# MiniMax-AI/VTP

Measured on AMD Instinct MI355X. Metric: images/sec/node VTP-B f16d64 256x256 train step, higher is better.
Workload: dtype bf16

## Files before the change

### vtp_amd/csrc/attention_resident.hip

```cpp
#include "common.h"
#include "diag.h"
#include <algorithm>
#include <cstdio>
#include "vtp_hip.h"

namespace vtp {

constexpr float LOG2E_R = 1.4426950408889634f;
constexpr float LN2_R = 0.6931471805599453f;
constexpr int RES_MAXN = 320;
constexpr int RES_SPLIT_COLS = 4;

struct AttnResArgs {
  const bf16 *q, *k, *v, *o, *d_o;
  bf16 *out, *dq, *dk, *dv;
  float* lse;
  float* delta;
  const bf16 *rope_sin, *rope_cos;
  int rope_prefix;
  int B, N, heads, npad;
  long sb, sn, sbo, sno;
  float scale;
  int stagger;
  unsigned long long* timing;
};

__device__ __forceinline__ void attn_stamp(const AttnResArgs& p, size_t wg, int lane, int wave, int i) {
  if (__builtin_expect(p.timing != nullptr, 0) && lane == 0) diag_stamp(p.timing, (wg * 16 + wave) * 8 + i);
}
__device__ __forceinline__ int grid_wg() { return (blockIdx.z * gridDim.y + blockIdx.y) * gridDim.x + blockIdx.x; }

__device__ __forceinline__ int swz_key(int r) { return (((r >> 1) & 1) << 2) | ((r >> 2) & 3); }

__device__ __forceinline__ void stage_resident(const bf16* __restrict__ base, long sn, int N, int npad, char* lds, int wave,
                                               int nwaves, int lane) {
  const int rr = lane >> 3, cp = lane & 7;
  for (int piece = wave; piece < (npad >> 3); piece += nwaves) {
    const int row = piece * 8 + rr;
    const int c = cp ^ swz_key(row);
    const bf16* src = base + (long)min(row, N - 1) * sn + c * 8;
    __builtin_amdgcn_global_load_lds((const __attribute__((address_space(1))) void*)src,
                                     (__attribute__((address_space(3))) void*)(lds + piece * 1024), 16, 0, 0);
  }
}

__device__ __forceinline__ bf16x8 frag_row(const char* lds, int row0, int ks, int lane) {
  const int r = row0 + (lane & 31);
  return *(const bf16x8*)(lds + r * 128 + (((2 * ks + (lane >> 5)) ^ swz_key(r)) << 4));
}
__device__ __forceinline__ bf16x8 frag_tr(const char* lds, int dblk, int row0, int ks, int lane) {
  const int i = lane & 15, g = (lane >> 4) & 1, hi = lane >> 5;
  const int r = row0 + ks * 16 + hi * 4 + (i >> 2);
  const int col = dblk * 32 + g * 16 + (i & 3) * 4;
  const char* p0 = lds + r * 128 + (((col >> 3) ^ swz_key(r)) << 4) + ((col & 7) << 1);
  const char* p1 = lds + (r + 8) * 128 + (((col >> 3) ^ swz_key(r + 8)) << 4) + ((col & 7) << 1);
  bf16x4 lo = __builtin_amdgcn_ds_read_tr16_b64_v4bf16((__attribute__((address_space(3))) bf16x4*)p0);
  bf16x4 hi4 = __builtin_amdgcn_ds_read_tr16_b64_v4bf16((__attribute__((address_space(3))) bf16x4*)p1);
  return __builtin_shufflevector(lo, hi4, 0, 1, 2, 3, 4, 5, 6, 7);
}

__device__ __forceinline__ int row_part(int lane) {
  const int r = lane & 31;
  return r * 128 + (((lane >> 5) ^ swz_key(r)) << 4);
}
__device__ __forceinline__ int tr_part(int lane, int half) {
  const int i = lane & 15, g = (lane >> 4) & 1, hi = lane >> 5;
  const int r = hi * 4 + (i >> 2) + 8 * half;
  const int col = g * 16 + (i & 3) * 4;
  return r * 128 + (((col >> 3) ^ swz_key(r)) << 4) + ((col & 7) << 1);
}
__device__ __forceinline__ int lds_addr(int lane_part, int uniform_part) {
  int a;
  asm("v_add_u32 %0, %1, %2" : "=v"(a) : "s"(uniform_part), "v"(lane_part));
  return a;
}
__device__ __forceinline__ bf16x8 frag_row_at(int addr) { return *(const __attribute__((address_space(3))) bf16x8*)(size_t)addr; }
__device__ __forceinline__ bf16x8 frag_tr_at(int addr0, int addr1, int ks) {
  bf16x4 lo = __builtin_amdgcn_ds_read_tr16_b64_v4bf16((__attribute__((address_space(3))) bf16x4*)(size_t)(addr0 + ks * 2048));
  bf16x4 hi4 = __builtin_amdgcn_ds_read_tr16_b64_v4bf16((__attribute__((address_space(3))) bf16x4*)(size_t)(addr1 + ks * 2048));
  return __builtin_shufflevector(lo, hi4, 0, 1, 2, 3, 4, 5, 6, 7);
}

__device__ __forceinline__ bf16x8 pack8r(const f32x16& a, int base) {
  f32x4 x = {a[base], a[base + 1], a[base + 2], a[base + 3]}, y = {a[base + 4], a[base + 5], a[base + 6], a[base + 7]};
  bf16x4 xb = __builtin_convertvector(x, bf16x4), yb = __builtin_convertvector(y, bf16x4);
  return __builtin_shufflevector(xb, yb, 0, 1, 2, 3, 4, 5, 6, 7);
}
__device__ __forceinline__ void zero16r(f32x16& a) {
#pragma unroll
  for (int r = 0; r < 16; ++r) a[r] = 0.f;
}
__device__ __forceinline__ void wait_all_dma() { asm volatile("s_waitcnt vmcnt(0)" ::: "memory"); }
__device__ __forceinline__ void wait_vmcnt_upto(int n) {
  switch (n) {
    case 0: asm volatile("s_waitcnt vmcnt(0)" ::: "memory"); break;
    case 1: asm volatile("s_waitcnt vmcnt(1)" ::: "memory"); break;
    case 2: asm volatile("s_waitcnt vmcnt(2)" ::: "memory"); break;
    case 3: asm volatile("s_waitcnt vmcnt(3)" ::: "memory"); break;
    case 4: asm volatile("s_waitcnt vmcnt(4)" ::: "memory"); break;
    case 5: asm volatile("s_waitcnt vmcnt(5)" ::: "memory"); break;
    case 6: asm volatile("s_waitcnt vmcnt(6)" ::: "memory"); break;
    case 7: asm volatile("s_waitcnt vmcnt(7)" ::: "memory"); break;
    case 8: asm volatile("s_waitcnt vmcnt(8)" ::: "memory"); break;
    case 9: asm volatile("s_waitcnt vmcnt(9)" ::: "memory"); break;
    case 10: asm volatile("s_waitcnt vmcnt(10)" ::: "memory"); break;
    case 11: asm volatile("s_waitcnt vmcnt(11)" ::: "memory"); break;
    case 12: asm volatile("s_waitcnt vmcnt(12)" ::: "memory"); break;
    case 13: asm volatile("s_waitcnt vmcnt(13)" ::: "memory"); break;
    case 14: asm volatile("s_waitcnt vmcnt(14)" ::: "memory"); break;
    case 15: asm volatile("s_waitcnt vmcnt(15)" ::: "memory"); break;
    case 16: asm volatile("s_waitcnt vmcnt(16)" ::: "memory"); break;
    case 17: asm volatile("s_waitcnt vmcnt(17)" ::: "memory"); break;
    case 18: asm volatile("s_waitcnt vmcnt(18)" ::: "memory"); break;
    case 19: asm volatile("s_waitcnt vmcnt(19)" ::: "memory"); break;
    case 20: asm volatile("s_waitcnt vmcnt(20)" ::: "memory"); break;
    case 21: asm volatile("s_waitcnt vmcnt(21)" ::: "memory"); break;
    case 22: asm volatile("s_waitcnt vmcnt(22)" ::: "memory"); break;
    case 23: asm volatile("s_waitcnt vmcnt(23)" ::: "memory"); break;
    case 24: asm volatile("s_waitcnt vmcnt(24)" ::: "memory"); break;
    case 25: asm volatile("s_waitcnt vmcnt(25)" ::: "memory"); break;
    case 26: asm volatile("s_waitcnt vmcnt(26)" ::: "memory"); break;
    case 27: asm volatile("s_waitcnt vmcnt(27)" ::: "memory"); break;
    case 28: asm volatile("s_waitcnt vmcnt(28)" ::: "memory"); break;
    case 29: asm volatile("s_waitcnt vmcnt(29)" ::: "memory"); break;
    case 30: asm volatile("s_waitcnt vmcnt(30)" ::: "memory"); break;
    case 31: asm volatile("s_waitcnt vmcnt(31)" ::: "memory"); break;
    case 32: asm volatile("s_waitcnt vmcnt(32)" ::: "memory"); break;
    default: asm volatile("s_waitcnt vmcnt(0)" ::: "memory"); break;
  }
}

__device__ __forceinline__ void store_grad_pair(bf16* row, int d0, f32x4 lo, f32x4 hi, const bf16* sin_t, const bf16* cos_t, long t) {
  bf16x4 a4 = __builtin_convertvector(lo, bf16x4), b4 = __builtin_convertvector(hi, bf16x4);
  if (sin_t) {
    const bf16x4 c1 = *(const bf16x4*)(cos_t + t + d0), c2 = *(const bf16x4*)(cos_t + t + d0 + 32);
    const bf16x4 s1 = *(const bf16x4*)(sin_t + t + d0), s2 = *(const bf16x4*)(sin_t + t + d0 + 32);
    bf16x4 o1, o2;
#pragma unroll
    for (int e = 0; e < 4; ++e) {
      const float a = bf2f(a4[e]), b = bf2f(b4[e]);
      o1[e] = f2bf(bf2f(f2bf(a * bf2f(c1[e]))) + bf2f(f2bf(b * bf2f(s2[e]))));
      o2[e] = f2bf(bf2f(f2bf(b * bf2f(c2[e]))) + bf2f(f2bf(-a * bf2f(s1[e]))));
    }
    a4 = o1;
    b4 = o2;
  }
  *(bf16x4*)(row + d0) = a4;
  *(bf16x4*)(row + d0 + 32) = b4;
}

__global__ __launch_bounds__(640) void attn_fwd_res_kernel(const AttnResArgs p) {
  extern __shared__ __attribute__((aligned(16))) char smem[];
  char* Ks = smem;
  char* Vs = smem + p.npad * 128;
  const int lane = threadIdx.x & 63, wave = __builtin_amdgcn_readfirstlane(threadIdx.x >> 6), nwaves = blockDim.x >> 6, hi = lane >> 5;
  const int h = blockIdx.x, b = blockIdx.y;
// ... 534 lines not shown
      dk[db] = __builtin_amdgcn_mfma_f32_32x32x16_bf16(frag_tr_at(tq0, tq1, 0), d0, dk[db], 0, 0, 0);
      dk[db] = __builtin_amdgcn_mfma_f32_32x32x16_bf16(frag_tr_at(tq0, tq1, 1), d1, dk[db], 0, 0, 0);
    }
  }
  stamp(2);
  if (ki < p.N) {
  bf16* krow = p.dk + (long)b * p.sb + (long)ki * p.sn + h * 64;
  bf16* vrow = p.dv + (long)b * p.sb + (long)ki * p.sn + h * 64;
  const bool rot = p.rope_sin && ki >= p.rope_prefix;
  const long t = (long)(ki - p.rope_prefix) * 64;
#pragma unroll
  for (int g = 0; g < 4; ++g) {
    f32x4 lo, hv, c0, c1;
#pragma unroll
    for (int e = 0; e < 4; ++e) {
      lo[e] = dk[0][4 * g + e];
      hv[e] = dk[1][4 * g + e];
      c0[e] = dv[0][4 * g + e];
      c1[e] = dv[1][4 * g + e];
    }
    store_grad_pair(krow, 8 * g + 4 * hi, lo, hv, rot ? p.rope_sin : nullptr, p.rope_cos, t);
    store_grad_pair(vrow, 8 * g + 4 * hi, c0, c1, nullptr, nullptr, 0);
  }
  }
  stamp(3);
}

constexpr int PB_WAVES = 8;
constexpr int PB_XROWS = 2;

__device__ __forceinline__ int stage_image_asm(const bf16* base, long sn, int N, int npad, unsigned img_off, int wave, int nwaves,
                                               int lane) {
  int n = 0;
  for (int piece = wave; piece < (npad >> 3); piece += nwaves, ++n) stage_piece_asm(base, sn, N, piece, img_off, lane);
  return n;
}

__device__ __forceinline__ void dq_step(const bf16x8 (&qf)[4], const bf16x8 (&dof)[4], f32x16 (&dq)[2], const int (&rpart)[4],
                                        const int (&tpart)[2][2], int koff, int img, f32x2 sc2v, f32x2 nlse, f32x2 scv, f32x2 ndlt,
                                        int key0, int N, bool mask, int hi) {
  f32x16 s, dp;
  zero16r(s);
  zero16r(dp);
#pragma unroll
  for (int ks = 0; ks < 4; ++ks) {
    s = __builtin_amdgcn_mfma_f32_32x32x16_bf16(frag_row_at(lds_addr(rpart[ks], koff)), qf[ks], s, 0, 0, 0);
    dp = __builtin_amdgcn_mfma_f32_32x32x16_bf16(frag_row_at(lds_addr(rpart[ks], koff + img)), dof[ks], dp, 0, 0, 0);
  }
#pragma unroll
  for (int i = 0; i < 8; ++i) {
    f32x2 e = {s[2 * i], s[2 * i + 1]}, g = {dp[2 * i], dp[2 * i + 1]};
    e = __builtin_elementwise_fma(e, sc2v, nlse);
    g = __builtin_elementwise_fma(g, scv, ndlt);
    e[0] = fast_exp2(e[0]);
    e[1] = fast_exp2(e[1]);
    e *= g;
    s[2 * i] = e[0];
    s[2 * i + 1] = e[1];
  }
  if (mask) {
#pragma unroll
    for (int r = 0; r < 16; ++r)
      if (key0 + (r & 3) + 8 * (r >> 2) + 4 * hi >= N) s[r] = 0.f;
  }
  const bf16x8 d0 = pack8r(s, 0), d1 = pack8r(s, 8);
#pragma unroll
  for (int db = 0; db < 2; ++db) {
    const int t0 = lds_addr(tpart[db][0], koff), t1 = lds_addr(tpart[db][1], koff);
    dq[db] = __builtin_amdgcn_mfma_f32_32x32x16_bf16(frag_tr_at(t0, t1, 0), d0, dq[db], 0, 0, 0);
    dq[db] = __builtin_amdgcn_mfma_f32_32x32x16_bf16(frag_tr_at(t0, t1, 1), d1, dq[db], 0, 0, 0);
  }
}

__device__ __forceinline__ float row_delta(const bf16x8 (&of)[4], const bf16x8 (&dof)[4]) {
  float dlt = 0.f;
#pragma unroll
  for (int ks = 0; ks < 4; ++ks)
#pragma unroll
    for (int e = 0; e < 8; ++e) dlt += bf2f(of[ks][e]) * bf2f(dof[ks][e]);
  return dlt + __shfl_xor(dlt, 32, 64);
}

__device__ __forceinline__ void dkv_step(const bf16x8 (&kf)[4], const bf16x8 (&vf)[4], f32x16 (&dk)[2], f32x16 (&dv)[2],
                                         const int (&rpart)[4], const int (&tpart)[2][2], int qoff, int img, const float* lse_s,
                                         const float* dlt_s, f32x2 sc2v, f32x2 scv, int q0, int N, bool mask, int hi) {
  f32x16 s, dp;
  zero16r(s);
  zero16r(dp);
#pragma unroll
  for (int ks = 0; ks < 4; ++ks) {
    s = __builtin_amdgcn_mfma_f32_32x32x16_bf16(frag_row_at(lds_addr(rpart[ks], qoff)), kf[ks], s, 0, 0, 0);
    dp = __builtin_amdgcn_mfma_f32_32x32x16_bf16(frag_row_at(lds_addr(rpart[ks], qoff + img)), vf[ks], dp, 0, 0, 0);
  }
  f32x16 pr;
#pragma unroll
  for (int g = 0; g < 4; ++g) {
    const f32x4 l4 = *(const f32x4*)(lse_s + q0 + 8 * g + 4 * hi);
    const f32x4 d4 = *(const f32x4*)(dlt_s + q0 + 8 * g + 4 * hi);
#pragma unroll
    for (int e2 = 0; e2 < 2; ++e2) {
      const int r = 4 * g + 2 * e2;
      f32x2 e = {s[r], s[r + 1]}, gq = {dp[r], dp[r + 1]};
      e = __builtin_elementwise_fma(e, sc2v, f32x2{l4[2 * e2], l4[2 * e2 + 1]});
      gq = __builtin_elementwise_fma(gq, scv, f32x2{d4[2 * e2], d4[2 * e2 + 1]});
      e[0] = fast_exp2(e[0]);
      e[1] = fast_exp2(e[1]);
      if (mask) {
        if (q0 + 8 * g + 4 * hi + 2 * e2 >= N) e[0] = 0.f;
        if (q0 + 8 * g + 4 * hi + 2 * e2 + 1 >= N) e[1] = 0.f;
      }
      pr[r] = e[0];
      pr[r + 1] = e[1];
      e *= gq;
      s[r] = e[0];
      s[r + 1] = e[1];
    }
  }
  const bf16x8 p0 = pack8r(pr, 0), p1 = pack8r(pr, 8), d0 = pack8r(s, 0), d1 = pack8r(s, 8);
#pragma unroll
  for (int db = 0; db < 2; ++db) {
    const int tq0 = lds_addr(tpart[db][0], qoff), tq1 = lds_addr(tpart[db][1], qoff);
    const int tg0 = lds_addr(tpart[db][0], qoff + img), tg1 = lds_addr(tpart[db][1], qoff + img);
    dv[db] = __builtin_amdgcn_mfma_f32_32x32x16_bf16(frag_tr_at(tg0, tg1, 0), p0, dv[db], 0, 0, 0);
    dv[db] = __builtin_amdgcn_mfma_f32_32x32x16_bf16(frag_tr_at(tg0, tg1, 1), p1, dv[db], 0, 0, 0);
    dk[db] = __builtin_amdgcn_mfma_f32_32x32x16_bf16(frag_tr_at(tq0, tq1, 0), d0, dk[db], 0, 0, 0);
    dk[db] = __builtin_amdgcn_mfma_f32_32x32x16_bf16(frag_tr_at(tq0, tq1, 1), d1, dk[db], 0, 0, 0);
  }
}

__device__ __forceinline__ void put_slot(float* slot, const f32x16 (&acc)[2], int hi) {
#pragma unroll
  for (int db = 0; db < 2; ++db)
#pragma unroll
    for (int g = 0; g < 4; ++g) {
      f32x4 v;
#pragma unroll
      for (int e = 0; e < 4; ++e) v[e] = acc[db][4 * g + e];
      *(f32x4*)(slot + 32 * db + 8 * g + 4 * hi) = v;
    }
}
__device__ __forceinline__ void store_acc_rows(bf16* row, const f32x16 (&acc)[2], int hi, const bf16* sin_t, const bf16* cos_t, long t) {
#pragma unroll
  for (int g = 0; g < 4; ++g) {
    f32x4 lo, hv;
#pragma unroll
    for (int e = 0; e < 4; ++e) {
      lo[e] = acc[0][4 * g + e];
      hv[e] = acc[1][4 * g + e];
    }
    store_grad_pair(row, 8 * g + 4 * hi, lo, hv, sin_t, cos_t, t);
  }
}

template <int W>
__global__ __launch_bounds__(64 * W) void attn_bwd_fused_kernel(const AttnResArgs p) {
  extern __shared__ __attribute__((aligned(16))) char smem[];
  const int lane = threadIdx.x & 63, wave = threadIdx.x >> 6, hi = lane >> 5;
  const int img = p.npad * 128, nb = p.npad >> 5, last = nb - 1;
  const bool odd = nb > W;
  const int nx = odd ? p.N - 32 * W : 0;
  const int QO = 0, KO = img, VO = 2 * img, GO = 3 * img;
  float* lse_s = (float*)(smem + 4 * img);
  float* dlt_s = lse_s + p.npad;
  float* xq = dlt_s + p.npad;
  float* xk = xq + (W + 1) * PB_XROWS * 64;
  float* xv = xk + (W + 1) * PB_XROWS * 64;
  const int hid = blockIdx.x, b = hid / p.heads, h = hid - b * p.heads;
  auto stamp = [&p, lane, wave, hid](int i) { attn_stamp(p, hid, lane, wave, i); };
  stamp(0);
  stage_image_asm(p.q + (long)b * p.sb + h * 64, p.sn, p.N, p.npad, QO, wave, W, lane);
  stage_image_asm(p.d_o + (long)b * p.sbo + h * 64, p.sno, p.N, p.npad, GO, wave, W, lane);
  stage_image_asm(p.k + (long)b * p.sb + h * 64, p.sn, p.N, p.npad, KO, wave, W, lane);
  stage_image_asm(p.v + (long)b * p.sb + h * 64, p.sn, p.N, p.npad, VO, wave, W, lane);
  const float sc2 = p.scale * LOG2E_R;
  const f32x2 sc2v = {sc2, sc2}, scv = {p.scale, p.scale};
  int rpart[4], tpart[2][2];
#pragma unroll
  for (int ks = 0; ks < 4; ++ks) rpart[ks] = row_part(lane) ^ (ks << 5);
#pragma unroll
  for (int db = 0; db < 2; ++db)
#pragma unroll
    for (int hf = 0; hf < 2; ++hf) tpart[db][hf] = tr_part(lane, hf) ^ (db << 6);
  const long srow0 = ((long)b * p.heads + h) * p.N;
  const int ri = wave * 32 + (lane & 31);
  const int rx = 32 * W + (lane & 31);
  bf16x8 of[4], of2[4];
  float lse_raw, lse_raw2 = 0.f;
  {
    const int qc = min(ri, p.N - 1);
    const bf16* orow = p.o + (long)b * p.sbo + h * 64 + (long)qc * p.sno + hi * 8;
#pragma unroll
    for (int ks = 0; ks < 4; ++ks) of[ks] = *(const bf16x8*)(orow + ks * 16);
    lse_raw = p.lse[srow0 + qc];
    if (odd) {
      const int qc2 = min(rx, p.N - 1);
      const bf16* orow2 = p.o + (long)b * p.sbo + h * 64 + (long)qc2 * p.sno + hi * 8;
#pragma unroll
      for (int ks = 0; ks < 4; ++ks) of2[ks] = *(const bf16x8*)(orow2 + ks * 16);
      lse_raw2 = p.lse[srow0 + qc2];
    }
  }
  wait_all_dma();
  __syncthreads();
  stamp(1);
  {
    bf16x8 qf[4], dof[4];
    const int own = __builtin_amdgcn_readfirstlane(wave * 4096);
#pragma unroll
    for (int ks = 0; ks < 4; ++ks) {
      qf[ks] = frag_row_at(lds_addr(rpart[ks], QO + own));
      dof[ks] = frag_row_at(lds_addr(rpart[ks], GO + own));
    }
    const float dlt = row_delta(of, dof);
    if (hi == 0) {
      lse_s[ri] = -lse_raw * LOG2E_R;
      dlt_s[ri] = -dlt * p.scale;
      if (ri < p.N) p.delta[srow0 + ri] = dlt;
    }
    {
      const float lse2 = lse_raw * LOG2E_R;
      const f32x2 nlse = {-lse2, -lse2}, ndlt = {-dlt * p.scale, -dlt * p.scale};
      f32x16 dq[2];
      zero16r(dq[0]);
      zero16r(dq[1]);
      for (int kb = 0; kb < nb; ++kb)
        dq_step(qf, dof, dq, rpart, tpart, __builtin_amdgcn_readfirstlane(KO + kb * 4096), img, sc2v, nlse, scv, ndlt, kb * 32, p.N,
                kb == last && (p.N & 31), hi);
      if (ri < p.N) {
        const bool rot = p.rope_sin && ri >= p.rope_prefix;
        store_acc_rows(p.dq + (long)b * p.sb + (long)ri * p.sn + h * 64, dq, hi, rot ? p.rope_sin : nullptr, p.rope_cos,
                       (long)(ri - p.rope_prefix) * 64);
      }
    }
    if (odd) {
      const int ox = __builtin_amdgcn_readfirstlane(W * 4096);
#pragma unroll
      for (int ks = 0; ks < 4; ++ks) {
        qf[ks] = frag_row_at(lds_addr(rpart[ks], QO + ox));
        dof[ks] = frag_row_at(lds_addr(rpart[ks], GO + ox));
      }
      const float dlt2 = row_delta(of2, dof);
      if (wave == 0 && hi == 0) {
        lse_s[rx] = -lse_raw2 * LOG2E_R;
        dlt_s[rx] = -dlt2 * p.scale;
        if (rx < p.N) p.delta[srow0 + rx] = dlt2;
      }
      const float lse2 = lse_raw2 * LOG2E_R;
      const f32x2 nlse = {-lse2, -lse2}, ndlt = {-dlt2 * p.scale, -dlt2 * p.scale};
      for (int kb = wave; kb < nb; kb += W) {
        f32x16 dqx[2];
        zero16r(dqx[0]);
        zero16r(dqx[1]);
        dq_step(qf, dof, dqx, rpart, tpart, __builtin_amdgcn_readfirstlane(KO + kb * 4096), img, sc2v, nlse, scv, ndlt, kb * 32, p.N,
                kb == last && (p.N & 31), hi);
        if ((lane & 31) < nx) put_slot(xq + (kb * PB_XROWS + (lane & 31)) * 64, dqx, hi);
      }
    }
  }
  __syncthreads();
  stamp(2);
  if (odd && (int)threadIdx.x < nx * 8) {
    const int row = threadIdx.x >> 3, d0 = 4 * (threadIdx.x & 7), qrow = 32 * W + row;
    f32x4 lo = {0.f, 0.f, 0.f, 0.f}, hv = {0.f, 0.f, 0.f, 0.f};
    for (int kb = 0; kb < nb; ++kb) {
      lo += *(const f32x4*)(xq + (kb * PB_XROWS + row) * 64 + d0);
      hv += *(const f32x4*)(xq + (kb * PB_XROWS + row) * 64 + 32 + d0);
    }
    const bool rot = p.rope_sin && qrow >= p.rope_prefix;
    store_grad_pair(p.dq + (long)b * p.sb + (long)qrow * p.sn + h * 64, d0, lo, hv, rot ? p.rope_sin : nullptr, p.rope_cos,
                    (long)(qrow - p.rope_prefix) * 64);
  }
  {
    bf16x8 kf[4], vf[4];
    const int own = __builtin_amdgcn_readfirstlane(wave * 4096);
#pragma unroll
    for (int ks = 0; ks < 4; ++ks) {
      kf[ks] = frag_row_at(lds_addr(rpart[ks], KO + own));
      vf[ks] = frag_row_at(lds_addr(rpart[ks], VO + own));
    }
    {
      f32x16 dk[2], dv[2];
      zero16r(dk[0]);
      zero16r(dk[1]);
      zero16r(dv[0]);
      zero16r(dv[1]);
      for (int qb = 0; qb < nb; ++qb)
        dkv_step(kf, vf, dk, dv, rpart, tpart, __builtin_amdgcn_readfirstlane(QO + qb * 4096), GO - QO, lse_s, dlt_s, sc2v, scv, qb * 32,
                 p.N, qb == last && (p.N & 31), hi);
      if (ri < p.N) {
        const bool rot = p.rope_sin && ri >= p.rope_prefix;
        store_acc_rows(p.dk + (long)b * p.sb + (long)ri * p.sn + h * 64, dk, hi, rot ? p.rope_sin : nullptr, p.rope_cos,
                       (long)(ri - p.rope_prefix) * 64);
        store_acc_rows(p.dv + (long)b * p.sb + (long)ri * p.sn + h * 64, dv, hi, nullptr, nullptr, 0);
      }
    }
    if (odd) {
      const int ox = __builtin_amdgcn_readfirstlane(W * 4096);
#pragma unroll
      for (int ks = 0; ks < 4; ++ks) {
        kf[ks] = frag_row_at(lds_addr(rpart[ks], KO + ox));
        vf[ks] = frag_row_at(lds_addr(rpart[ks], VO + ox));
      }
      for (int qb = wave; qb < nb; qb += W) {
        f32x16 dkx[2], dvx[2];
        zero16r(dkx[0]);
        zero16r(dkx[1]);
        zero16r(dvx[0]);
        zero16r(dvx[1]);
        dkv_step(kf, vf, dkx, dvx, rpart, tpart, __builtin_amdgcn_readfirstlane(QO + qb * 4096), GO - QO, lse_s, dlt_s, sc2v, scv,
                 qb * 32, p.N, qb == last && (p.N & 31), hi);
        if ((lane & 31) < nx) {
          put_slot(xk + (qb * PB_XROWS + (lane & 31)) * 64, dkx, hi);
          put_slot(xv + (qb * PB_XROWS + (lane & 31)) * 64, dvx, hi);
        }
      }
    }
  }
  if (odd) {
    __syncthreads();
    if ((int)threadIdx.x < nx * 8) {
      const int row = threadIdx.x >> 3, d0 = 4 * (threadIdx.x & 7), krow_i = 32 * W + row;
      f32x4 lo = {0.f, 0.f, 0.f, 0.f}, hv = lo, c0 = lo, c1 = lo;
      for (int qb = 0; qb < nb; ++qb) {
        lo += *(const f32x4*)(xk + (qb * PB_XROWS + row) * 64 + d0);
        hv += *(const f32x4*)(xk + (qb * PB_XROWS + row) * 64 + 32 + d0);
        c0 += *(const f32x4*)(xv + (qb * PB_XROWS + row) * 64 + d0);
        c1 += *(const f32x4*)(xv + (qb * PB_XROWS + row) * 64 + 32 + d0);
      }
      const bool rot = p.rope_sin && krow_i >= p.rope_prefix;
      store_grad_pair(p.dk + (long)b * p.sb + (long)krow_i * p.sn + h * 64, d0, lo, hv, rot ? p.rope_sin : nullptr, p.rope_cos,
                      (long)(krow_i - p.rope_prefix) * 64);
      store_grad_pair(p.dv + (long)b * p.sb + (long)krow_i * p.sn + h * 64, d0, c0, c1, nullptr, nullptr, 0);
    }
  }
  stamp(3);
}

static int res_waves_per_block(int nw, int groups) {
  return (groups <= 512 && nw >= 4) ? (nw + 1) / 2 : nw;
}

template <typename K>
static void set_lds(K kern, int bytes) {
  hipFuncSetAttribute((const void*)kern, hipFuncAttributeMaxDynamicSharedMemorySize, bytes);
}

static unsigned long long* g_attn_timing = nullptr;
static int g_attn_wpb = 0;
static int g_attn_lds_pad = 0;
static int g_attn_stagger = 0;

int attn_resident_fwd(const void* q, const void* k, const void* v, void* o, float* lse, int B, int N, int heads, long sb,
                      long sn, long sbo, long sno, float scale, hipStream_t s) {
  AttnResArgs a = {};
  a.q = (const bf16*)q; a.k = (const bf16*)k; a.v = (const bf16*)v; a.out = (bf16*)o; a.lse = lse;
  a.B = B; a.N = N; a.heads = heads; a.npad = (N + 31) / 32 * 32; a.sb = sb; a.sn = sn; a.sbo = sbo; a.sno = sno; a.scale = scale;
  a.timing = g_attn_timing;
  static bool attr = false;
  if (!attr) {
    set_lds(attn_fwd_res_kernel, 2 * RES_MAXN * 128);
    set_lds(attn_fwd_res2_kernel, 2 * RES_MAXN * 128 + 5 * RES_SPLIT_COLS * 2 * 34 * 4);
    attr = true;
  }
  {
    const int ntiles = a.npad / 32, cols = N - 32 * (ntiles - 1);
    const bool odd = (ntiles & 1) && ntiles > 1;
    if ((!odd || cols <= RES_SPLIT_COLS) && ntiles / 2 <= 4) {
      const int waves = std::max(1, ntiles / 2);
      const int lds = 2 * a.npad * 128 + (odd ? waves * cols * 2 * 34 * 4 : 0);
      if (a.timing) {
        int occ = -1;
        (void)hipOccupancyMaxActiveBlocksPerMultiprocessor(&occ, attn_fwd_res2_kernel, 64 * waves, lds);
        fprintf(stderr, "[attn timing] workgroups per CU by the runtime's count: %d (lds %d B, %d waves)\n", occ, lds, waves);
      }
      hipLaunchKernelGGL(attn_fwd_res2_kernel, dim3(heads, B), dim3(64 * waves), lds, s, a);
      return check_launch("attn_fwd_resident2");
    }
  }
  const int nw = a.npad / 32, wpb = res_waves_per_block(nw, heads * B);
  hipLaunchKernelGGL(attn_fwd_res_kernel, dim3(heads, B, (nw + wpb - 1) / wpb), dim3(64 * wpb), 2 * a.npad * 128, s, a);
  return check_launch("attn_fwd_resident");
}

int attn_resident_bwd(const void* q, const void* k, const void* v, const void* o, const void* d_o, const float* lse,
                      float* delta, void* dq, void* dk, void* dv, const void* rope_sin, const void* rope_cos, int rope_prefix,
                      int B, int N, int heads, long sb, long sn, long sbo, long sno, float scale, hipStream_t s) {
  AttnResArgs a = {};
  a.q = (const bf16*)q; a.k = (const bf16*)k; a.v = (const bf16*)v; a.o = (const bf16*)o; a.d_o = (const bf16*)d_o;
  a.lse = (float*)lse; a.delta = delta; a.dq = (bf16*)dq; a.dk = (bf16*)dk; a.dv = (bf16*)dv;
  a.rope_sin = (const bf16*)rope_sin; a.rope_cos = (const bf16*)rope_cos; a.rope_prefix = rope_prefix;
  a.B = B; a.N = N; a.heads = heads; a.npad = (N + 31) / 32 * 32; a.sb = sb; a.sn = sn; a.sbo = sbo; a.sno = sno; a.scale = scale;
  a.timing = g_attn_timing;
  a.stagger = g_attn_stagger;
  static bool attr = false;
  if (!attr) {
    set_lds(attn_bwd_dq_res_kernel, 2 * RES_MAXN * 128 + 32768);
    set_lds(attn_bwd_dkv_res_kernel, 2 * RES_MAXN * 128 + 8 * RES_MAXN + 32768);
    attr = true;
  }
  const int nw = a.npad / 32;
  auto fits = [&](int W) { return nw == W || (nw == W + 1 && N - 32 * W <= PB_XROWS); };
  const bool off32 = (long)N * sn * 2 < (1L << 31) && (long)N * sno * 2 < (1L << 31);
  if (g_attn_wpb == 0 && off32 && (fits(PB_WAVES) || fits(2))) {
    auto lds_of = [](int npad, int W) { return 4 * npad * 128 + 8 * npad + 3 * (W + 1) * PB_XROWS * 256; };
    static bool attr_p = false;
    if (!attr_p) {
      set_lds(attn_bwd_fused_kernel<PB_WAVES>, lds_of(32 * (PB_WAVES + 1), PB_WAVES));
      set_lds(attn_bwd_fused_kernel<2>, lds_of(32 * 3, 2));
      attr_p = true;
    }
    if (fits(PB_WAVES))
      hipLaunchKernelGGL(attn_bwd_fused_kernel<PB_WAVES>, dim3(B * heads), dim3(64 * PB_WAVES), lds_of(a.npad, PB_WAVES), s, a);
    else
      hipLaunchKernelGGL(attn_bwd_fused_kernel<2>, dim3(B * heads), dim3(128), lds_of(a.npad, 2), s, a);
    return check_launch("attn_bwd_fused");
  }
  const int wpb = g_attn_wpb > 0 ? std::min(g_attn_wpb, nw) : res_waves_per_block(nw, heads * B);
  const dim3 grid(heads, B, (nw + wpb - 1) / wpb), block(64 * wpb);
  if (a.timing) {
    int o1 = -1, o2 = -1;
    (void)hipOccupancyMaxActiveBlocksPerMultiprocessor(&o1, attn_bwd_dq_res_kernel, block.x, 2 * a.npad * 128);
    (void)hipOccupancyMaxActiveBlocksPerMultiprocessor(&o2, attn_bwd_dkv_res_kernel, block.x, 2 * a.npad * 128 + 8 * a.npad);
    fprintf(stderr, "[attn timing] workgroups per CU by the runtime's count: dQ %d, dK/dV %d (%d waves, lds %d / %d B)\n", o1, o2,
            (int)block.x / 64, 2 * a.npad * 128, 2 * a.npad * 128 + 8 * a.npad);
  }
  hipLaunchKernelGGL(attn_bwd_dq_res_kernel, grid, block, 2 * a.npad * 128 + g_attn_lds_pad, s, a);
  if (a.timing) a.timing += (size_t)grid.x * grid.y * grid.z * 16 * 8;
  hipLaunchKernelGGL(attn_bwd_dkv_res_kernel, grid, block, 2 * a.npad * 128 + 8 * a.npad + g_attn_lds_pad, s, a);
  return check_launch("attn_bwd_resident");
}

}

extern "C" int vtp_attn_debug(void* timing, int lds_pad, int waves_per_wg, int stagger_ticks) {
  const bool off = timing == nullptr && lds_pad == 0 && waves_per_wg == 0 && stagger_ticks == 0;
  if (!off && !vtp::diag_allowed("vtp_attn_debug")) return VTP_ERR_ARG;
  VTP_REQUIRE(lds_pad >= 0 && stagger_ticks >= 0, "vtp_attn_debug: negative LDS pad / stagger");
  vtp::g_attn_timing = (unsigned long long*)timing;
  vtp::g_attn_lds_pad = lds_pad;
  vtp::g_attn_wpb = waves_per_wg;
  vtp::g_attn_stagger = stagger_ticks;
  return VTP_OK;
}
```

Baseline: 769.2.

## Handle odd tail rows with scalar side path instead of a padded extra tile

Adds a specialised fused attention-backward kernel for sequences with one partial 32-row tile beyond the resident waves (e.g. 256 tokens plus prefix). Instead of staging and running MFMA over a full padded tile for the few leftover rows, the tail rows are kept in small LDS buffers and handled with dot-product and axpy side computations, plus small MFMA reductions that scatter their contributions. This avoids the wasted padded-tile work and masking in every step, at the cost of more code, extra LDS, and serialised per-row work on wave 0 and wave 1. It is enabled by default and can be turned off with an environment variable.

```diff
diff --git a/vtp_amd/csrc/attention_resident.hip b/vtp_amd/csrc/attention_resident.hip
--- a/vtp_amd/csrc/attention_resident.hip
+++ b/vtp_amd/csrc/attention_resident.hip
@@ -2,6 +2,7 @@
 #include "diag.h"
 #include <algorithm>
 #include <cstdio>
+#include <cstdlib>
 #include "vtp_hip.h"
 
 namespace vtp {
@@ -842,26 +843,125 @@
   }
 }
 
-template <int W>
-__global__ __launch_bounds__(64 * W) void attn_bwd_fused_kernel(const AttnResArgs p) {
-  extern __shared__ __attribute__((aligned(16))) char smem[];
+enum { XM_Q = 0, XM_K = 1, XM_V = 2, XM_G = 3 };
+
+__device__ __forceinline__ float side_dot(const bf16x8 (&rf)[4], const bf16* xr, int m, int x, int hi) {
+  float acc = 0.f;
+#pragma unroll
+  for (int ks = 0; ks < 4; ++ks) {
+    const bf16x8 o = *(const bf16x8*)(xr + (m * PB_XROWS + x) * 64 + 16 * ks + 8 * hi);
+#pragma unroll
+    for (int e = 0; e < 4; ++e)
+      acc = __builtin_amdgcn_fdot2_f32_bf16(bf16x2{rf[ks][2 * e], rf[ks][2 * e + 1]}, bf16x2{o[2 * e], o[2 * e + 1]}, acc, false);
+  }
+  return both_halves_sum(acc);
+}
+__device__ __forceinline__ void side_axpy(f32x16 (&acc)[2], float w, const float* xf, int m, int x, int hi) {
+#pragma unroll
+  for (int db = 0; db < 2; ++db)
+#pragma unroll
+    for (int g = 0; g < 4; ++g) {
+      const f32x4 v = *(const f32x4*)(xf + (m * PB_XROWS + x) * 64 + 32 * db + 8 * g + 4 * hi);
+#pragma unroll
+      for (int e = 0; e < 4; ++e) acc[db][4 * g + e] += w * v[e];
+    }
+}
+__device__ __forceinline__ void side_q(const bf16x8 (&qf)[4], const bf16x8 (&dof)[4], f32x16 (&dq)[2], float nlse, float ndlt, float sc2,
+                                       float scale, int nx, const bf16* xr, const float* xf, int hi, float (&dsx)[PB_XROWS],
+                                       float (&px)[PB_XROWS]) {
+#pragma unroll
+  for (int x = 0; x < PB_XROWS; ++x) {
+    dsx[x] = 0.f;
+    px[x] = 0.f;
+    if (x < nx) {
+      const float s = side_dot(qf, xr, XM_K, x, hi), dp = side_dot(dof, xr, XM_V, x, hi);
+      px[x] = fast_exp2(fmaf(s, sc2, nlse));
+      dsx[x] = px[x] * fmaf(dp, scale, ndlt);
+      side_axpy(dq, dsx[x], xf, XM_K, x, hi);
+    }
+  }
+}
+__device__ __forceinline__ void side_k(const bf16x8 (&kf)[4], const bf16x8 (&vf)[4], f32x16 (&dk)[2], f32x16 (&dv)[2], const float* lse_x,
+                                       const float* dlt_x, float sc2, float scale, int nx, const bf16* xr, const float* xf, int hi,
+                                       float (&dsx)[PB_XROWS]) {
+#pragma unroll
+  for (int x = 0; x < PB_XROWS; ++x) {
+    dsx[x] = 0.f;
+    if (x < nx) {
+      const float s = side_dot(kf, xr, XM_Q, x, hi), dp = side_dot(vf, xr, XM_G, x, hi);
+      const float pr = fast_exp2(fmaf(s, sc2, lse_x[x]));
+      dsx[x] = pr * fmaf(dp, scale, dlt_x[x]);
+      side_axpy(dk, dsx[x], xf, XM_Q, x, hi);
+      side_axpy(dv, pr, xf, XM_G, x, hi);
+    }
+  }
+}
+__device__ __forceinline__ void side_reduce(const float (&w)[PB_XROWS], float* bounce, int ioff, const int (&tpart)[2][2], float* slot,
+                                            int nx, int lane) {
+  const int c = lane & 31, hi = lane >> 5;
+  if (hi == 0) {
+#pragma unroll
+    for (int x = 0; x < PB_XROWS; ++x) bounce[x * 32 + c] = w[x];
+  }
+  __builtin_amdgcn_wave_barrier();
+  const float* src = bounce + min(c, PB_XROWS - 1) * 32 + 4 * hi;
+  f32x4 a[4];
+#pragma unroll
+  for (int j = 0; j < 4; ++j) {
+    a[j] = *(const f32x4*)(src + 8 * j);
+    if (c >= nx) a[j] = f32x4{0.f, 0.f, 0.f, 0.f};
+  }
+  __builtin_amdgcn_wave_barrier();
+  const bf16x4 b0 = __builtin_convertvector(a[0], bf16x4), b1 = __builtin_convertvector(a[1], bf16x4);
+  const bf16x4 b2 = __builtin_convertvector(a[2], bf16x4), b3 = __builtin_convertvector(a[3], bf16x4);
+  const bf16x8 w0 = __builtin_shufflevector(b0, b1, 0, 1, 2, 3, 4, 5, 6, 7), w1 = __builtin_shufflevector(b2, b3, 0, 1, 2, 3, 4, 5, 6, 7);
+  f32x16 acc[2];
+  zero16r(acc[0]);
+  zero16r(acc[1]);
+#pragma unroll
+  for (int db = 0; db < 2; ++db) {
+    const int t0 = lds_addr(tpart[db][0], ioff), t1 = lds_addr(tpart[db][1], ioff);
+    acc[db] = __builtin_amdgcn_mfma_f32_32x32x16_bf16(frag_tr_at(t0, t1, 0), w0, acc[db], 0, 0, 0);
+    acc[db] = __builtin_amdgcn_mfma_f32_32x32x16_bf16(frag_tr_at(t0, t1, 1), w1, acc[db], 0, 0, 0);
+  }
+  if (c < nx) put_slot(slot + c * 64, acc, hi);
+}
+
+template <int W, bool SB>
+__device__ __forceinline__ void attn_bwd_fused_body(const AttnResArgs& p, char* smem) {
   const int lane = threadIdx.x & 63, wave = threadIdx.x >> 6, hi = lane >> 5;
-  const int img = p.npad * 128, nb = p.npad >> 5, last = nb - 1;
-  const bool odd = nb > W;
-  const int nx = odd ? p.N - 32 * W : 0;
+  const int irows = SB ? 32 * W : p.npad;
+  const int img = irows * 128, nb = irows >> 5, last = nb - 1;
+  const bool odd = !SB && nb > W;
+  const int nx = (SB || odd) ? p.N - 32 * W : 0;
   const int QO = 0, KO = img, VO = 2 * img, GO = 3 * img;
   float* lse_s = (float*)(smem + 4 * img);
   float* dlt_s = lse_s + p.npad;
   float* xq = dlt_s + p.npad;
   float* xk = xq + (W + 1) * PB_XROWS * 64;
   float* xv = xk + (W + 1) * PB_XROWS * 64;
+  float* xf = xv + (W + 1) * PB_XROWS * 64;
+  bf16* xr = (bf16*)(xf + 4 * PB_XROWS * 64);
+  float* bounce = (float*)(xr + 4 * PB_XROWS * 64) + wave * 2 * PB_XROWS * 32;
   const int hid = blockIdx.x, b = hid / p.heads, h = hid - b * p.heads;
   auto stamp = [&p, lane, wave, hid](int i) { attn_stamp(p, hid, lane, wave, i); };
   stamp(0);
-  stage_image_asm(p.q + (long)b * p.sb + h * 64, p.sn, p.N, p.npad, QO, wave, W, lane);
-  stage_image_asm(p.d_o + (long)b * p.sbo + h * 64, p.sno, p.N, p.npad, GO, wave, W, lane);
-  stage_image_asm(p.k + (long)b * p.sb + h * 64, p.sn, p.N, p.npad, KO, wave, W, lane);
-  stage_image_asm(p.v + (long)b * p.sb + h * 64, p.sn, p.N, p.npad, VO, wave, W, lane);
+  stage_image_asm(p.q + (long)b * p.sb + h * 64, p.sn, p.N, irows, QO, wave, W, lane);
+  stage_image_asm(p.d_o + (long)b * p.sbo + h * 64, p.sno, p.N, irows, GO, wave, W, lane);
+  stage_image_asm(p.k + (long)b * p.sb + h * 64, p.sn, p.N, irows, KO, wave, W, lane);
+  stage_image_asm(p.v + (long)b * p.sb + h * 64, p.sn, p.N, irows, VO, wave, W, lane);
+  if (SB && (int)threadIdx.x < 4 * PB_XROWS * 8) {
+    const int m = threadIdx.x / (PB_XROWS * 8), x = (threadIdx.x >> 3) % PB_XROWS, c = threadIdx.x & 7;
+    if (x < nx) {
+      const bf16* src = m == XM_G ? p.d_o + (long)b * p.sbo + (long)(32 * W + x) * p.sno
+                                  : (m == XM_Q ? p.q : m == XM_K ? p.k : p.v) + (long)b * p.sb + (long)(32 * W + x) * p.sn;
+      const bf16x8 v = *(const bf16x8*)(src + h * 64 + c * 8);
+      const int at = (m * PB_XROWS + x) * 64 + c * 8;
+      *(bf16x8*)(xr + at) = v;
+      *(f32x4*)(xf + at) = f32x4{bf2f(v[0]), bf2f(v[1]), bf2f(v[2]), bf2f(v[3])};
+      *(f32x4*)(xf + at + 4) = f32x4{bf2f(v[4]), bf2f(v[5]), bf2f(v[6]), bf2f(v[7])};
+    }
+  }
   const float sc2 = p.scale * LOG2E_R;
   const f32x2 sc2v = {sc2, sc2}, scv = {p.scale, p.scale};
   int rpart[4], tpart[2][2];
@@ -882,7 +982,7 @@
 #pragma unroll
     for (int ks = 0; ks < 4; ++ks) of[ks] = *(const bf16x8*)(orow + ks * 16);
     lse_raw = p.lse[srow0 + qc];
-    if (odd) {
+    if (odd || (SB && wave == 0)) {
       const int qc2 = min(rx, p.N - 1);
       const bf16* orow2 = p.o + (long)b * p.sbo + h * 64 + (long)qc2 * p.sno + hi * 8;
 #pragma unroll
@@ -915,11 +1015,52 @@
       zero16r(dq[1]);
       for (int kb = 0; kb < nb; ++kb)
         dq_step(qf, dof, dq, rpart, tpart, __builtin_amdgcn_readfirstlane(KO + kb * 4096), img, sc2v, nlse, scv, ndlt, kb * 32, p.N,
-                kb == last && (p.N & 31), hi);
+                !SB && kb == last && (p.N & 31), hi);
+      float dsx[PB_XROWS], px[PB_XROWS];
+      if (SB) side_q(qf, dof, dq, -lse2, -dlt * p.scale, sc2, p.scale, nx, xr, xf, hi, dsx, px);
       if (ri < p.N) {
         const bool rot = p.rope_sin && ri >= p.rope_prefix;
         store_acc_rows(p.dq + (long)b * p.sb + (long)ri * p.sn + h * 64, dq, hi, rot ? p.rope_sin : nullptr, p.rope_cos,
                        (long)(ri - p.rope_prefix) * 64);
+      }
+      if (SB) {
+        side_reduce(dsx, bounce, QO + own, tpart, xk + wave * PB_XROWS * 64, nx, lane);
+        side_reduce(px, bounce + PB_XROWS * 32, GO + own, tpart, xv + wave * PB_XROWS * 64, nx, lane);
+      }
+    }
+    if (SB && wave == 0) {
+      const int c = lane & 31, x = min(c, nx - 1);
+#pragma unroll
+      for (int ks = 0; ks < 4; ++ks) {
+        qf[ks] = *(const bf16x8*)(xr + (XM_Q * PB_XROWS + x) * 64 + 16 * ks + 8 * hi);
+        dof[ks] = *(const bf16x8*)(xr + (XM_G * PB_XROWS + x) * 64 + 16 * ks + 8 * hi);
+      }
+      const float dlt2 = row_delta(of2, dof);
+      if (hi == 0 && c < nx) {
+        lse_s[rx] = -lse_raw2 * LOG2E_R;
+        dlt_s[rx] = -dlt2 * p.scale;
+        p.delta[srow0 + rx] = dlt2;
+      }
+      __builtin_amdgcn_wave_barrier();
+      float dsx[PB_XROWS], px[PB_XROWS];
+      f32x16 ax[2], bx[2];
+      zero16r(ax[0]);
+      zero16r(ax[1]);
+      side_q(qf, dof, ax, -lse_raw2 * LOG2E_R, -dlt2 * p.scale, sc2, p.scale, nx, xr, xf, hi, dsx, px);
+      if (c < nx) put_slot(xq + (W * PB_XROWS + c) * 64, ax, hi);
+#pragma unroll
+      for (int ks = 0; ks < 4; ++ks) {
+        qf[ks] = *(const bf16x8*)(xr + (XM_K * PB_XROWS + x) * 64 + 16 * ks + 8 * hi);
+        dof[ks] = *(const bf16x8*)(xr + (XM_V * PB_XROWS + x) * 64 + 16 * ks + 8 * hi);
+      }
+      zero16r(ax[0]);
+      zero16r(ax[1]);
+      zero16r(bx[0]);
+      zero16r(bx[1]);
+      side_k(qf, dof, ax, bx, lse_s + 32 * W, dlt_s + 32 * W, sc2, p.scale, nx, xr, xf, hi, dsx);
+      if (c < nx) {
+        put_slot(xk + (W * PB_XROWS + c) * 64, ax, hi);
+        put_slot(xv + (W * PB_XROWS + c) * 64, bx, hi);
       }
     }
     if (odd) {
@@ -949,17 +1090,36 @@
   }
   __syncthreads();
   stamp(2);
-  if (odd && (int)threadIdx.x < nx * 8) {
-    const int row = threadIdx.x >> 3, d0 = 4 * (threadIdx.x & 7), qrow = 32 * W + row;
-    f32x4 lo = {0.f, 0.f, 0.f, 0.f}, hv = {0.f, 0.f, 0.f, 0.f};
-    for (int kb = 0; kb < nb; ++kb) {
-      lo += *(const f32x4*)(xq + (kb * PB_XROWS + row) * 64 + d0);
-      hv += *(const f32x4*)(xq + (kb * PB_XROWS + row) * 64 + 32 + d0);
-    }
-    const bool rot = p.rope_sin && qrow >= p.rope_prefix;
-    store_grad_pair(p.dq + (long)b * p.sb + (long)qrow * p.sn + h * 64, d0, lo, hv, rot ? p.rope_sin : nullptr, p.rope_cos,
-                    (long)(qrow - p.rope_prefix) * 64);
-  }
+  auto store_xq = [&](int tid) {
+    if (tid < nx * 8) {
+      const int row = tid >> 3, d0 = 4 * (tid & 7), qrow = 32 * W + row;
+      f32x4 lo = {0.f, 0.f, 0.f, 0.f}, hv = {0.f, 0.f, 0.f, 0.f};
+      for (int kb = 0; kb < W + 1; ++kb) {
+        lo += *(const f32x4*)(xq + (kb * PB_XROWS + row) * 64 + d0);
+        hv += *(const f32x4*)(xq + (kb * PB_XROWS + row) * 64 + 32 + d0);
+      }
+      const bool rot = p.rope_sin && qrow >= p.rope_prefix;
+      store_grad_pair(p.dq + (long)b * p.sb + (long)qrow * p.sn + h * 64, d0, lo, hv, rot ? p.rope_sin : nullptr, p.rope_cos,
+                      (long)(qrow - p.rope_prefix) * 64);
+    }
+  };
+  auto store_xkv = [&](int tid) {
+    if (tid < nx * 8) {
+      const int row = tid >> 3, d0 = 4 * (tid & 7), krow_i = 32 * W + row;
+      f32x4 lo = {0.f, 0.f, 0.f, 0.f}, hv = lo, c0 = lo, c1 = lo;
+      for (int qb = 0; qb < W + 1; ++qb) {
+        lo += *(const f32x4*)(xk + (qb * PB_XROWS + row) * 64 + d0);
+        hv += *(const f32x4*)(xk + (qb * PB_XROWS + row) * 64 + 32 + d0);
+        c0 += *(const f32x4*)(xv + (qb * PB_XROWS + row) * 64 + d0);
+        c1 += *(const f32x4*)(xv + (qb * PB_XROWS + row) * 64 + 32 + d0);
+      }
+      const bool rot = p.rope_sin && krow_i >= p.rope_prefix;
+      store_grad_pair(p.dk + (long)b * p.sb + (long)krow_i * p.sn + h * 64, d0, lo, hv, rot ? p.rope_sin : nullptr, p.rope_cos,
+                      (long)(krow_i - p.rope_prefix) * 64);
+      store_grad_pair(p.dv + (long)b * p.sb + (long)krow_i * p.sn + h * 64, d0, c0, c1, nullptr, nullptr, 0);
+    }
+  };
+  if (odd) store_xq(threadIdx.x);
   {
     bf16x8 kf[4], vf[4];
     const int own = __builtin_amdgcn_readfirstlane(wave * 4096);
@@ -976,13 +1136,16 @@
       zero16r(dv[1]);
       for (int qb = 0; qb < nb; ++qb)
         dkv_step(kf, vf, dk, dv, rpart, tpart, __builtin_amdgcn_readfirstlane(QO + qb * 4096), GO - QO, lse_s, dlt_s, sc2v, scv, qb * 32,
-                 p.N, qb == last && (p.N & 31), hi);
+                 p.N, !SB && qb == last && (p.N & 31), hi);
+      float dsx[PB_XROWS];
+      if (SB) side_k(kf, vf, dk, dv, lse_s + 32 * W, dlt_s + 32 * W, sc2, p.scale, nx, xr, xf, hi, dsx);
       if (ri < p.N) {
         const bool rot = p.rope_sin && ri >= p.rope_prefix;
         store_acc_rows(p.dk + (long)b * p.sb + (long)ri * p.sn + h * 64, dk, hi, rot ? p.rope_sin : nullptr, p.rope_cos,
                        (long)(ri - p.rope_prefix) * 64);
         store_acc_rows(p.dv + (long)b * p.sb + (long)ri * p.sn + h * 64, dv, hi, nullptr, nullptr, 0);
       }
+      if (SB) side_reduce(dsx, bounce, KO + own, tpart, xq + wave * PB_XROWS * 64, nx, lane);
     }
     if (odd) {
       const int ox = __builtin_amdgcn_readfirstlane(W * 4096);
@@ -1006,24 +1169,23 @@
       }
     }
   }
-  if (odd) {
+  if (odd || SB) {
     __syncthreads();
-    if ((int)threadIdx.x < nx * 8) {
-      const int row = threadIdx.x >> 3, d0 = 4 * (threadIdx.x & 7), krow_i = 32 * W + row;
-      f32x4 lo = {0.f, 0.f, 0.f, 0.f}, hv = lo, c0 = lo, c1 = lo;
-      for (int qb = 0; qb < nb; ++qb) {
-        lo += *(const f32x4*)(xk + (qb * PB_XROWS + row) * 64 + d0);
-        hv += *(const f32x4*)(xk + (qb * PB_XROWS + row) * 64 + 32 + d0);
-        c0 += *(const f32x4*)(xv + (qb * PB_XROWS + row) * 64 + d0);
-        c1 += *(const f32x4*)(xv + (qb * PB_XROWS + row) * 64 + 32 + d0);
-      }
-      const bool rot = p.rope_sin && krow_i >= p.rope_prefix;
-      store_grad_pair(p.dk + (long)b * p.sb + (long)krow_i * p.sn + h * 64, d0, lo, hv, rot ? p.rope_sin : nullptr, p.rope_cos,
-                      (long)(krow_i - p.rope_prefix) * 64);
-      store_grad_pair(p.dv + (long)b * p.sb + (long)krow_i * p.sn + h * 64, d0, c0, c1, nullptr, nullptr, 0);
-    }
+    if (!SB) store_xkv(threadIdx.x);
+    else if (wave == 0) store_xq(lane);
+    else if (wave == 1) store_xkv(lane);
   }
   stamp(3);
+}
+
+template <int W>
+__global__ __launch_bounds__(64 * W) void attn_bwd_fused_kernel(const AttnResArgs p) {
+  extern __shared__ __attribute__((aligned(16))) char smem[];
+  attn_bwd_fused_body<W, false>(p, smem);
+}
+__global__ __launch_bounds__(64 * PB_WAVES) void attn_bwd_fused_odd_kernel(const AttnResArgs p) {
+  extern __shared__ __attribute__((aligned(16))) char smem[];
+  attn_bwd_fused_body<PB_WAVES, true>(p, smem);
 }
 
 static int res_waves_per_block(int nw, int groups) {
@@ -1039,6 +1201,11 @@
 static int g_attn_wpb = 0;
 static int g_attn_lds_pad = 0;
 static int g_attn_stagger = 0;
+
+static bool attn_odd_enabled() {
+  const char* e = getenv("VTP_ATTN_ODD");
+  return !(e && e[0] == '0' && e[1] == 0);
+}
 
 int attn_resident_fwd(const void* q, const void* k, const void* v, void* o, float* lse, int B, int N, int heads, long sb,
                       long sn, long sbo, long sno, float scale, hipStream_t s) {
@@ -1099,6 +1266,17 @@
       set_lds(attn_bwd_fused_kernel<2>, lds_of(32 * 3, 2));
       attr_p = true;
     }
+    if (nw == PB_WAVES + 1 && fits(PB_WAVES) && attn_odd_enabled()) {
+      constexpr int W = PB_WAVES;
+      const int lds = 4 * 32 * W * 128 + 8 * a.npad + 3 * (W + 1) * PB_XROWS * 256 + 4 * PB_XROWS * 64 * (4 + 2) + W * 2 * PB_XROWS * 32 * 4;
+      static bool attr_s = false;
+      if (!attr_s) {
+        set_lds(attn_bwd_fused_odd_kernel, lds);
+        attr_s = true;
+      }
+      hipLaunchKernelGGL(attn_bwd_fused_odd_kernel, dim3(B * heads), dim3(64 * W), lds, s, a);
+      return check_launch("attn_bwd_fused_odd");
+    }
     if (fits(PB_WAVES))
       hipLaunchKernelGGL(attn_bwd_fused_kernel<PB_WAVES>, dim3(B * heads), dim3(64 * PB_WAVES), lds_of(a.npad, PB_WAVES), s, a);
     else
```

Measured after the change: 774.4, median of 6. Within noise of the previous version (+0.7%).
